# pranoyr/attention-models

Measured on AMD Instinct MI355X. Metric: ViTVQGAN 256px train-step images/sec, higher is better.
Workload: dtype f32; 1 GPU; BASELINE.json configs[2]: ViTVQGAN dim=256 patch=8 img=256 depth=6+6 h=8 d=64 mlp=2048 (SwiGLU), codebook 8192x32; GAN train step (D phase + G phase, gradient penalty, per_loss_weight=0), Adam, clip 1.0; global_batch=32, batch_per_gpu=32, parallelism=dp1

## Files before the change

### attention-models_amd/amk/lib.py

```python
import ctypes
import os
import re

_HERE = os.path.dirname(os.path.abspath(__file__))
LIB_PATH = os.environ.get("AMK_LIB") or os.path.join(_HERE, "libamk.so")
HEADER_PATH = os.path.normpath(os.path.join(_HERE, "..", "..", "include", "amk.h"))

AMK_OK = 0

_c = ctypes
_P = _c.c_void_p
_I = _c.c_int
_L = _c.c_int64
_F = _c.c_float



class GemmDesc(_c.Structure):
    _fields_ = [("op", _c.c_int32), ("epilogue", _c.c_int32), ("m", _L),
                ("n", _c.c_int32), ("k", _c.c_int32), ("split", _c.c_int32), ("reserved", _c.c_int32),
                ("a", _P), ("a2", _P), ("w", _P), ("w2", _P), ("c", _P), ("c2", _P),
                ("lda", _L), ("lda2", _L), ("ldw", _L), ("ldw2", _L), ("ldc", _L), ("ldc2", _L),
                ("bias", _P), ("bias2", _P), ("resid", _P), ("ldr", _L),
                ("ln_mean", _P), ("ln_rstd", _P), ("ln_gamma", _P), ("ln_beta", _P),
                ("ab", _P), ("ldab", _L), ("gate", _P), ("ldg", _L), ("dbias", _P)]


GEMM_NT, GEMM_NN, GEMM_TN = 0, 1, 2
EPI_BIAS, EPI_RESID, EPI_SWIGLU, EPI_SWIGLU_BWD = 0, 1, 2, 3

SIGNATURES = {
    "amk_version": (_I, []),
    "amk_arch": (_c.c_char_p, []),
    "amk_last_error": (_c.c_char_p, []),
    "amk_attn_fwd": (_I, [_P] * 7 + [_I] * 5 + [_L] * 12 + [_F, _P]),
    "amk_attn_scores_bytes": (_L, [_I, _I, _I, _I]),
    "amk_attn_fwd_keep": (_I, [_P] * 8 + [_I] * 5 + [_L] * 12 + [_F, _P]),
    "amk_attn_fwd_x6_ws_bytes": (_L, [_I, _I, _I]),
    "amk_attn_fwd_x6": (_I, [_P] * 8 + [_I] * 5 + [_L] * 12 + [_F, _P]),
    "amk_attn_bwd_ws_floats": (_L, [_I, _I, _I, _I, _I]),
    "amk_attn_bwd": (_I, [_P] * 12 + [_I] * 5 + [_L] * 24 + [_F, _I, _P]),
    "amk_attn_bwd_kept": (_I, [_P] * 13 + [_I] * 5 + [_L] * 24 + [_F, _I, _P]),
    "amk_vq_num_partials": (_L, [_L]),
    "amk_vq_lookup_fwd": (_I, [_P, _P, _L, _I, _I, _I] + [_P] * 9 + [_P]),
    "amk_vq_lookup_bwd": (_I, [_P] * 7 + [_F, _L, _I, _I, _P, _P, _P]),
    "amk_vq_lookup_bwd_rows": (_I, [_P] * 7 + [_F, _L, _I, _I, _P, _P, _P]),
    "amk_vq_padded_codes": (_I, [_I, _I]),
    "amk_vq_gather": (_I, [_P, _P, _L, _I, _I, _P, _P, _P]),
    "amk_agent_num_chunks": (_I, [_I]),
    "amk_agent_ws_floats": (_L, [_I, _I, _I, _I, _I]),
    "amk_agent_num_chunks_dh": (_I, [_I, _I]),
    "amk_agent_ws_floats_dh": (_L, [_I, _I, _I, _I, _I, _I]),
    "amk_agent_attn_fwd": (_I, [_P] * 10 + [_I] * 5 + [_L] * 12 + [_F, _P]),
    "amk_agent_attn_bwd": (_I, [_P] * 14 + [_I] * 5 + [_L] * 21 + [_F, _P]),
    "amk_agent_conv_grad_reduce": (_I, [_P, _P, _L, _I, _P, _P, _P]),
    "amk_rowsum_num_partials": (_I, [_L]),
    "amk_add_layernorm_fwd": (_I, [_P, _P, _P, _P, _L, _I, _F, _P, _P, _P, _P, _P]),
    "amk_add_layernorm_bwd": (_I, [_P, _P, _P, _P, _P, _P, _L, _I, _P, _P, _P]),
    "amk_colsum": (_I, [_P, _L, _I, _P, _P]),
    "amk_swiglu_fwd": (_I, [_P, _L, _I, _P, _P]),
    "amk_swiglu_bwd": (_I, [_P, _P, _L, _I, _P, _P]),
    "amk_geglu_fwd": (_I, [_P, _L, _I, _P, _P]),
    "amk_geglu_bwd": (_I, [_P, _P, _L, _I, _P, _P]),
    "amk_opt_num_partials": (_I, []),
    "amk_sumsq_partials": (_I, [_P, _L, _P, _P]),
    "amk_adam_flat_step": (_I, [_P] * 4 + [_L, _P, _P, _P, _I] + [_F] * 6 + [_I, _P, _P]),
    "amk_adam_flat_step_shadow": (_I, [_P] * 4 + [_L, _P, _P, _P, _I] + [_F] * 6 + [_I, _P, _P, _P]),
    "amk_gemm_x6_planes_bytes": (_L, [_I, _I]),
    "amk_gemm_x6_split": (_I, [_P, _L, _I, _I, _P, _P]),
    "amk_gemm_x6_nt": (_I, [_P, _L, _P, _P, _P, _L, _I, _I, _I, _P]),
    "amk_gemm_f32_ws_bytes": (_L, [_c.POINTER(GemmDesc)]),
    "amk_gemm_f32": (_I, [_c.POINTER(GemmDesc), _P, _L, _P]),
    "amk_row_stats": (_I, [_P, _L, _I, _F, _P, _P, _P]),
    "amk_attn_bf16_fwd": (_I, [_P] * 7 + [_I] * 5 + [_L] * 12 + [_F, _P]),
    "amk_attn_bf16_bwd_ws_floats": (_L, [_I, _I, _I, _I]),
    "amk_attn_bf16_bwd": (_I, [_P] * 12 + [_I] * 5 + [_L] * 24 + [_F, _P]),
    "amk_swiglu_bf16_fwd": (_I, [_P, _L, _I, _P, _P]),
    "amk_swiglu_bf16_bwd": (_I, [_P, _P, _L, _I, _P, _P]),
    "amk_add_layernorm_mixed_fwd": (_I, [_P, _I, _P, _P, _P, _L, _I, _F, _P, _P, _P, _P, _P]),
    "amk_add_layernorm_mixed_bwd": (_I, [_P, _I, _P, _P, _P, _P, _P, _L, _I, _P, _P, _P, _P]),
    "amk_gemm_bf16": (_I, [_I, _I, _P, _L, _P, _L, _P, _P, _L, _P, _L, _L, _I, _I, _P]),
    "amk_gemm_bf16_swiglu_bwd": (_I, [_P, _L, _P, _L, _P, _L, _P, _L, _L, _I, _I, _P]),
    "amk_gemm_tn_bf16_ws_bytes": (_L, [_L, _I, _I]),
    "amk_gemm_tn_bf16": (_I, [_P, _L, _P, _L, _P, _L, _P, _L, _I, _I, _P, _L, _P]),
    "amk_sample_step": (_I, [_P, _P, _F, _P, _c.c_uint64, _c.c_uint64, _F, _L, _I, _I, _P, _F, _P, _P, _P]),
    "amk_moe_route_ws_ints": (_L, [_L, _I, _I]),
    "amk_moe_route": (_I, [_P, _L, _I, _I] + [_P] * 8),
    "amk_grouped_gemm_nt": (_I, [_P, _L, _I, _P, _P, _P, _P, _L, _I, _I, _I, _P, _P]),
    "amk_grouped_gemm_nn": (_I, [_P, _L, _I, _P, _P, _P, _P, _L, _I, _I, _I, _P, _P]),
    "amk_grouped_gemm_nt_acc": (_I, [_P, _L, _I, _P, _P, _P, _P, _L, _I, _I, _I, _P, _I, _P]),
    "amk_grouped_gemm_nn_acc": (_I, [_P, _L, _I, _P, _P, _P, _P, _L, _I, _I, _I, _P, _I, _P]),
    "amk_grouped_gemm_wgrad": (_I, [_P, _L, _I, _P, _L, _I, _P, _P, _P, _L, _I, _I, _I, _P, _P, _P]),
    "amk_moe_combine": (_I, [_P, _P, _P, _L, _I, _I, _I, _P, _P]),
    "amk_moe_expert_sums": (_I, [_P, _L, _I, _P, _P, _L, _I, _I, _I, _P, _P]),
    "amk_moe_topk": (_I, [_P, _L, _I, _I, _P, _P, _P]),
    "amk_moe_route_distinct": (_I, [_P, _L, _I, _I, _P, _P, _P, _P]),
    "amk_moe_combine_rows": (_I, [_P, _P, _P, _L, _I, _I, _I, _I, _I, _P, _P]),
    "amk_moe_gate_grad_rows": (_I, [_P, _P, _P, _P, _L, _I, _I, _I, _I, _I, _P, _P]),
    "amk_moe_gate_grad": (_I, [_P, _P, _P, _P, _L, _I, _I, _I, _I, _P, _P]),
}

_lib = None


def declared_symbols(header_path=HEADER_PATH):
    text = open(header_path).read()
    text = re.sub(r"/\*.*?\*/", "", text, flags=re.S)
    return sorted(set(re.findall(r"\b(amk_[a-z0-9_]+)\s*\(", text)))


def load():
    global _lib
    if _lib is not None:
        return _lib
    if not os.path.exists(LIB_PATH):
        raise RuntimeError(
            f"{LIB_PATH} is missing: build it with `python -c 'import __graft_entry__ as g; g.build()'` "
            "(hipcc --offload-arch=gfx950). amk has no CPU or eager fallback."
        )
    lib = ctypes.CDLL(LIB_PATH)
    for name, (res, args) in SIGNATURES.items():
        fn = getattr(lib, name)
        fn.restype = res
        fn.argtypes = args
    arch = lib.amk_arch().decode()
    if arch != "gfx950":
        raise RuntimeError(f"libamk.so was built for {arch}, expected gfx950")
    _lib = lib
    return lib


def check(rc, what):
    if rc != AMK_OK:
        msg = load().amk_last_error().decode()
        raise RuntimeError(f"{what} failed with code {rc}: {msg}")
```

### attention-models_amd/amk/models/discriminator.py

```python
import contextlib

import torch
import torch.nn as nn
import torch.nn.functional as F
from torch.nn.grad import conv2d_input, conv2d_weight

_INPUT_GRAD_ONLY = False


@contextlib.contextmanager
def input_grad_only():
    global _INPUT_GRAD_ONLY
    old, _INPUT_GRAD_ONLY = _INPUT_GRAD_ONLY, True
    try:
        yield
    finally:
        _INPUT_GRAD_ONLY = old


class _ConvDataGrad(torch.autograd.Function):

    @staticmethod
    def forward(ctx, gy, weight, x_shape, stride, padding):
        ctx.save_for_backward(gy, weight)
        ctx.cfg = (stride, padding)
        return conv2d_input(x_shape, weight, gy, stride=stride, padding=padding)

    @staticmethod
    def backward(ctx, ggx):
        gy, weight = ctx.saved_tensors
        stride, padding = ctx.cfg
        ggx = ggx.contiguous()
        ggy = F.conv2d(ggx, weight, None, stride, padding) if ctx.needs_input_grad[0] else None
        gw = conv2d_weight(ggx, weight.shape, gy, stride=stride, padding=padding) if ctx.needs_input_grad[1] else None
        return ggy, gw, None, None, None


class _Conv(torch.autograd.Function):
    @staticmethod
    def forward(ctx, x, weight, bias, stride, padding):
        ctx.save_for_backward(x, weight)
        ctx.cfg = (stride, padding, bias is not None)
        return F.conv2d(x, weight, bias, stride, padding)

    @staticmethod
    def backward(ctx, gy):
        x, weight = ctx.saved_tensors
        stride, padding, has_bias = ctx.cfg
        gy = gy.contiguous()
        gx = _ConvDataGrad.apply(gy, weight, x.shape, stride, padding) if ctx.needs_input_grad[0] else None
        gw = gb = None
        if not _INPUT_GRAD_ONLY:
            if ctx.needs_input_grad[1]:
                gw = conv2d_weight(x, weight.shape, gy, stride=stride, padding=padding)
            if has_bias and ctx.needs_input_grad[2]:
                gb = gy.sum((0, 2, 3))
        return gx, gw, gb, None, None


class Conv2d(nn.Conv2d):

    def forward(self, x):
        if self.groups != 1 or self.dilation != (1, 1) or self.padding_mode != "zeros" or isinstance(self.padding, str):
            return super().forward(x)
        if torch.is_autocast_enabled():
            if self.in_channels < 8 and x.is_cuda:
                with torch.autocast("cuda", enabled=False):
                    return _Conv.apply(x.float(), self.weight, self.bias, self.stride, self.padding)
            return super().forward(x)
        return _Conv.apply(x, self.weight, self.bias, self.stride, self.padding)


class NLayerDiscriminator(nn.Module):
    def __init__(self, input_nc=3, ndf=64, n_layers=3):
        super().__init__()
        widths = [ndf * min(2 ** i, 8) for i in range(n_layers + 1)]
        layers = [Conv2d(input_nc, widths[0], 4, stride=2, padding=1), nn.LeakyReLU(0.2, True)]
        for i in range(1, n_layers + 1):
            stride = 2 if i < n_layers else 1
            layers += [
                Conv2d(widths[i - 1], widths[i], 4, stride=stride, padding=1, bias=False),
                nn.BatchNorm2d(widths[i]),
                nn.LeakyReLU(0.2, True),
            ]
        layers.append(Conv2d(widths[-1], 1, 4, stride=1, padding=1))
        self.model = nn.Sequential(*layers)

    def forward(self, x):
        return self.model(x)
```

### attention-models_amd/amk/ops.py

```python
import ctypes
import os
import weakref

import torch
from torch.autograd.function import once_differentiable

from . import lib as _lib

_NULL = ctypes.c_void_p(0)


def _ptr(t):
    return ctypes.c_void_p(t.data_ptr()) if t is not None else _NULL


def _stream():
    return ctypes.c_void_p(torch.cuda.current_stream().cuda_stream)


KERNEL_EVENTS = None


class _timed:

# ... 1106 lines not shown
        rc = L.amk_gemm_x6_nt(_ptr(a2), a2.stride(0), _ptr(planes), _ptr(bias), _ptr(c), N, M, N, K, _stream())
    _lib.check(rc, "amk_gemm_x6_nt")
    return c


def _x6_ok(x, weight):
    K = weight.shape[1]
    if K % 4 or x.numel() == 0 or x.data_ptr() % 16 or weight.data_ptr() % 16:
        return False
    if x.stride(-1) != 1 or (x.dim() >= 2 and x.stride(-2) % 4):
        return False
    return x.numel() * 4 < 0x7ffffff0 and weight.numel() * 8 < 0x7ffffff0


class _LinearX6(torch.autograd.Function):

    @staticmethod
    def forward(ctx, x, weight, bias):
        _require_device(x, weight, bias)
        x2 = x.reshape(-1, x.shape[-1])
        ctx.save_for_backward(x2, weight)
        ctx.x_shape = x.shape
        ctx.has_bias = bias is not None
        return gemm_x6_nt(x2, weight, bias).view(*x.shape[:-1], weight.shape[0])

    @staticmethod
    @once_differentiable
    def backward(ctx, dy):
        x2, weight = ctx.saved_tensors
        dy2 = dy.contiguous().view(-1, dy.shape[-1])
        dx = dw = db = None
        if ctx.needs_input_grad[0]:
            N = weight.shape[0]
            if N % 4 == 0:
                dx = gemm_x6_nt(dy2, weight.t().contiguous()).view(ctx.x_shape)
            else:
                dx = dy2.mm(weight).view(ctx.x_shape)
        if ctx.needs_input_grad[1]:
            dw = dy2.t().mm(x2)
        if ctx.has_bias and ctx.needs_input_grad[2]:
            db = colsum(dy2)
        return dx, dw, db


DENSE_MODE = os.environ.get("AMK_DENSE", "auto")


DENSE_AUTO_MAX_K = int(os.environ.get("AMK_DENSE_MAX_K", "512"))


def _dense_ok(x, *weights):
    if DENSE_MODE == "lib" or torch.is_autocast_enabled() or not x.is_cuda or x.dtype != torch.float32 or x.numel() == 0:
        return False
    if x.shape[-1] % 4 or x.shape[-1] < 128:
        return False
    if DENSE_MODE == "auto" and x.shape[-1] > DENSE_AUTO_MAX_K:
        return False
    return all(w.dtype == torch.float32 and w.shape[0] % 4 == 0 and w.shape[0] >= 128 and w.is_contiguous() for w in weights)


def _nn_plain(dy2, weight):
    from . import dense

    if DENSE_MODE == "amk":
        return dense.gemm_nn(dy2, weight)
    return dy2.mm(weight)


def _claim(p):
    ref = getattr(p, "_amk_reducer", None) if p is not None else None
    red = ref() if ref is not None else None
    if red is None:
        return None, None
    view = red.claim(p)
    return (red, view) if view is not None else (None, None)


class _DenseLinear(torch.autograd.Function):

    @staticmethod
    def forward(ctx, x, weight, bias):
        from . import dense

        x2 = x.reshape(-1, x.shape[-1])
        ctx.save_for_backward(x2, weight)
        ctx.x_shape = x.shape
        ctx.has_bias = bias is not None
        ctx.params = (weight, bias)
        if DENSE_MODE == "auto" and weight.shape[0] < 512:
            return torch.nn.functional.linear(x, weight, bias)
        return dense.gemm_nt(x2, weight, bias).view(*x.shape[:-1], weight.shape[0])

    @staticmethod
    @once_differentiable
    def backward(ctx, dy):
        from . import dense

        x2, weight = ctx.saved_tensors
        dy2 = dy.reshape(-1, dy.shape[-1])
        dx = dw = db = None
        if ctx.needs_input_grad[0]:
            dx = _nn_plain(dy2, weight).view(ctx.x_shape)
        if ctx.needs_input_grad[1] or (ctx.has_bias and ctx.needs_input_grad[2]):
            want_b = ctx.has_bias and ctx.needs_input_grad[2]
            (wr, wv), (br, bv) = _claim(ctx.params[0]), (_claim(ctx.params[1]) if want_b else (None, None))
            dw, _, db = dense.gemm_tn(dy2, x2, want_bias=want_b, out=wv, bias_out=bv)
            if wv is not None:
                wr.wrote(ctx.params[0])
                dw = None
            if bv is not None:
                br.wrote(ctx.params[1])
                db = None
        return dx, dw, db


def _tn_into(tn, y, x, weight, bias):
    (wr, wv), (br, bv) = _claim(weight), _claim(bias)
    res = tn(y, x, want_bias=bias is not None, out=wv, bias_out=bv)
    dw, db = res[0], res[-1]
    if wv is not None:
        wr.wrote(weight)
        dw = None
    if bv is not None:
        br.wrote(bias)
        db = None
    return dw, db


class _DenseLinear2(torch.autograd.Function):

    @staticmethod
    def forward(ctx, x, wa, wb):
        from . import dense

        x2 = x.reshape(-1, x.shape[-1])
        ctx.save_for_backward(x2, wa, wb)
        ctx.x_shape = x.shape
        ctx.params = (wa, wb)
        a, b = dense.gemm_nt(x2, wa, None, w2=wb)
        return a.view(*x.shape[:-1], wa.shape[0]), b.view(*x.shape[:-1], wb.shape[0])

    @staticmethod
    @once_differentiable
    def backward(ctx, da, db_):
        from . import dense

        x2, wa, wb = ctx.saved_tensors
        da2 = da.reshape(-1, da.shape[-1])
        db2 = db_.reshape(-1, db_.shape[-1])
        dx = dense.gemm_nn(da2, wa, a2=db2, w2=wb).view(ctx.x_shape) if ctx.needs_input_grad[0] else None
        dwa = dwb = None
        if ctx.needs_input_grad[1] or ctx.needs_input_grad[2]:
            (ar, av), (br, bv) = _claim(ctx.params[0]), _claim(ctx.params[1])
            dwa, dwb, _ = dense.gemm_tn(da2, x2, y2=db2, out=av, out2=bv)
            if av is not None:
                ar.wrote(ctx.params[0])
                dwa = None
            if bv is not None:
                br.wrote(ctx.params[1])
                dwb = None
        return dx, dwa, dwb


class _SwiGLUFFN(torch.autograd.Function):

    @staticmethod
    def forward(ctx, x, w12, b12, w3, b3):
        from . import dense

        x2 = x.reshape(-1, x.shape[-1])
        need = any(ctx.needs_input_grad)
        gate, ab = dense.gemm_nt_swiglu(x2, w12, b12, keep_ab=need)
        out = dense.gemm_nt(gate, w3, b3)
        if need:
            ctx.save_for_backward(x2, w12, w3, ab, gate)
        ctx.x_shape = x.shape
        ctx.has_bias = (b12 is not None, b3 is not None)
        ctx.params = (w12, b12, w3, b3)
        return out.view(*x.shape[:-1], w3.shape[0])

    @staticmethod
    @once_differentiable
    def backward(ctx, dout):
        from . import dense

        x2, w12, w3, ab, gate = ctx.saved_tensors
        d2 = dout.reshape(-1, dout.shape[-1])
        d_ab = dense.gemm_nn(d2, w3, swiglu_ab=ab)
        dw3, db3 = _tn_into(dense.gemm_tn, d2, gate, ctx.params[2], ctx.params[3] if ctx.has_bias[1] else None)
        dx = _nn_plain(d_ab, w12).view(ctx.x_shape) if ctx.needs_input_grad[0] else None
        dw12, db12 = _tn_into(dense.gemm_tn, d_ab, x2, ctx.params[0], ctx.params[1] if ctx.has_bias[0] else None)
        return dx, dw12, db12, dw3, db3


MIXED_WGRAD = os.environ.get("AMK_MIXED_WGRAD", "1") == "1"


def _w16(t):
    if t is None:
        return None
    shadow = getattr(t, "_amk_bf16", None)
    if shadow is not None and t._version == t._amk_bf16_version:
        return shadow
    return t.to(torch.bfloat16)


class _LinearMixed(torch.autograd.Function):

    @staticmethod
    def forward(ctx, x, weight, bias):
        x16, w16 = x.to(torch.bfloat16), _w16(weight)
        ctx.save_for_backward(x16, w16)
        ctx.has_bias, ctx.x_dtype = bias is not None, x.dtype
        ctx.params = (weight, bias)
        return torch.nn.functional.linear(x16, w16, _w16(bias))

    @staticmethod
    @once_differentiable
    def backward(ctx, dy):
        from . import dense

        x16, w16 = ctx.saved_tensors
        dy2 = dy.reshape(-1, dy.shape[-1])
        dx = dy2.mm(w16).view(x16.shape).to(ctx.x_dtype) if ctx.needs_input_grad[0] else None
        dw, db = _tn_into(dense.gemm_tn_bf16, dy2, x16.reshape(-1, x16.shape[-1]), ctx.params[0], ctx.params[1])
        return dx, dw, db


def _mixed_linear_ok(x, weight):
    return (MIXED_WGRAD and x.is_cuda and torch.get_autocast_dtype("cuda") == torch.bfloat16 and torch.is_grad_enabled()
            and weight.requires_grad and weight.dtype == torch.float32 and x.dtype in (torch.float32, torch.bfloat16)
            and weight.shape[0] % 8 == 0 and weight.shape[1] % 8 == 0 and x.numel() > 0)


def linear(x, weight, bias=None):
    if torch.is_autocast_enabled():
        if _mixed_linear_ok(x, weight):
            return _LinearMixed.apply(x, weight, bias)
        return torch.nn.functional.linear(x, weight, bias)
    if GEMM_MODE == "bf16x6" and _x6_ok(x, weight):
        return _LinearX6.apply(x, weight, bias)
    if _dense_ok(x, weight):
        return _DenseLinear.apply(x, weight, bias)
    if bias is None:
        return torch.nn.functional.linear(x, weight)
    return _BiasLinear.apply(x, weight, bias)


def linear2(x, wa, wb):
    if GEMM_MODE != "bf16x6" and _dense_ok(x, wa, wb) and wa.shape[0] % 128 == 0:
        return _DenseLinear2.apply(x, wa, wb)
    return linear(x, wa), linear(x, wb)


class _SwiGLUFFNMixed(torch.autograd.Function):

    @staticmethod
    def forward(ctx, x, w12, b12, w3, b3):
        from . import dense

        x16 = x.to(torch.bfloat16).reshape(-1, x.shape[-1])
        w12h, w3h = _w16(w12), _w16(w3)
        g, ab = dense.gemm_nt_swiglu_bf16(x16, w12h, b12)
        y = torch.nn.functional.linear(g, w3h, _w16(b3))
        ctx.save_for_backward(x16, ab, g, w12h, w3h)
        ctx.x_shape, ctx.x_dtype, ctx.bias = x.shape, x.dtype, (b12 is not None, b3 is not None)
        ctx.params = (w12, b12, w3, b3)
        return y.view(*x.shape[:-1], w3.shape[0])

    @staticmethod
    @once_differentiable
    def backward(ctx, dy):
        from . import dense

        x16, ab, g, w12h, w3h = ctx.saved_tensors
        dy2 = dy.reshape(-1, dy.shape[-1])
        dw3, db3 = _tn_into(dense.gemm_tn_bf16, dy2, g, ctx.params[2], ctx.params[3])
        dab = dense.gemm_nn_swiglu_bwd_bf16(dy2, w3h, ab)
        dw12, db12 = _tn_into(dense.gemm_tn_bf16, dab, x16, ctx.params[0], ctx.params[1])
        dx = dab.mm(w12h).view(ctx.x_shape).to(ctx.x_dtype) if ctx.needs_input_grad[0] else None
        return dx, dw12, db12, dw3, db3


def swiglu_ffn(x, w12, b12, w3, b3):
    if torch.is_autocast_enabled() and w12.shape[0] % 16 == 0 and w12.shape[0] >= 1024:
        if _mixed_linear_ok(x, w12) and _mixed_linear_ok(x, w3) and w3.requires_grad:
            with torch.autocast("cuda", enabled=False):
                return _SwiGLUFFNMixed.apply(x, w12, b12, w3, b3)
        no_grad = not torch.is_grad_enabled() or not any(
            t is not None and t.requires_grad for t in (x, w12, b12, w3, b3))
        if (MIXED_WGRAD and no_grad and x.is_cuda and torch.get_autocast_dtype("cuda") == torch.bfloat16
                and w12.dtype == torch.float32 and x.dtype in (torch.float32, torch.bfloat16) and w12.shape[1] % 8 == 0 and x.numel()):
            from . import dense

            g, _ = dense.gemm_nt_swiglu_bf16(x.to(torch.bfloat16).reshape(-1, x.shape[-1]), _w16(w12), b12, keep_ab=False)
            return torch.nn.functional.linear(g, _w16(w3), _w16(b3)).view(*x.shape[:-1], w3.shape[0])
    if GEMM_MODE != "bf16x6" and _dense_ok(x, w12) and w3.shape[1] % 4 == 0 and w3.shape[0] % 4 == 0 and w3.is_contiguous():
        return _SwiGLUFFN.apply(x, w12, b12, w3, b3)
    ab = linear(x, w12, b12)
    if ab.shape[-1] % 8 == 0:
        return linear(swiglu(ab), w3, b3)
    a, b = ab.chunk(2, dim=-1)
    return linear(torch.nn.functional.silu(a) * b, w3, b3)
```

### include/amk.h

```cpp
#ifndef AMK_H_
#define AMK_H_

#include <stdint.h>

#ifdef __cplusplus
extern "C" {
#endif

#define AMK_VERSION 140

enum {
  AMK_OK = 0,
  AMK_EINVAL = -1,
  AMK_EUNSUPPORTED = -2,
  AMK_ELAUNCH = -3
};

int amk_version(void);
const char* amk_arch(void);
const char* amk_last_error(void);

int amk_attn_fwd(const float* q, const float* k, const float* v, float* o, float* stats,
                 const uint8_t* key_mask, const uint8_t* causal_mask,
                 int B, int H, int I, int J, int D,
                 int64_t q_sb, int64_t q_st, int64_t q_sh,
                 int64_t k_sb, int64_t k_st, int64_t k_sh,
                 int64_t v_sb, int64_t v_st, int64_t v_sh,
                 int64_t o_sb, int64_t o_st, int64_t o_sh,
                 float scale, void* stream);

int64_t amk_attn_scores_bytes(int B, int H, int I, int J);
int amk_attn_fwd_keep(const float* q, const float* k, const float* v, float* o, float* stats, float* scores,
                      const uint8_t* key_mask, const uint8_t* causal_mask,
                      int B, int H, int I, int J, int D,
                      int64_t q_sb, int64_t q_st, int64_t q_sh,
                      int64_t k_sb, int64_t k_st, int64_t k_sh,
                      int64_t v_sb, int64_t v_st, int64_t v_sh,
                      int64_t o_sb, int64_t o_st, int64_t o_sh,
                      float scale, void* stream);

int64_t amk_attn_fwd_x6_ws_bytes(int B, int H, int J);
int amk_attn_fwd_x6(const float* q, const float* k, const float* v, float* o, float* stats, void* ws,
                    const uint8_t* key_mask, const uint8_t* causal_mask,
                    int B, int H, int I, int J, int D,
                    int64_t q_sb, int64_t q_st, int64_t q_sh,
                    int64_t k_sb, int64_t k_st, int64_t k_sh,
                    int64_t v_sb, int64_t v_st, int64_t v_sh,
                    int64_t o_sb, int64_t o_st, int64_t o_sh,
                    float scale, void* stream);

#define AMK_ATTN_BWD_DELTA 1
#define AMK_ATTN_BWD_DKDV 2
#define AMK_ATTN_BWD_DQ 4
#define AMK_ATTN_BWD_FUSED 8
#define AMK_ATTN_BWD_ALL 7
#define AMK_ATTN_BWD_FAST 9
#define AMK_ATTN_BWD_KEYS128 16
#define AMK_ATTN_BWD_KEYS256 32
#define AMK_ATTN_BWD_DQ_REPRO 64
#define AMK_ATTN_BWD_FAST_REPRO 73
int64_t amk_attn_bwd_ws_floats(int B, int H, int I, int J, int stages);
int amk_attn_bwd(const float* q, const float* k, const float* v, const float* o,
                 const float* stats, const float* d_o,
                 float* dq, float* dk, float* dv, float* delta_ws,
                 const uint8_t* key_mask, const uint8_t* causal_mask,
                 int B, int H, int I, int J, int D,
                 int64_t q_sb, int64_t q_st, int64_t q_sh,
                 int64_t k_sb, int64_t k_st, int64_t k_sh,
                 int64_t v_sb, int64_t v_st, int64_t v_sh,
                 int64_t o_sb, int64_t o_st, int64_t o_sh,
                 int64_t do_sb, int64_t do_st, int64_t do_sh,
                 int64_t dq_sb, int64_t dq_st, int64_t dq_sh,
                 int64_t dk_sb, int64_t dk_st, int64_t dk_sh,
                 int64_t dv_sb, int64_t dv_st, int64_t dv_sh,
                 float scale, int stages, void* stream);
int amk_attn_bwd_kept(const float* scores, const float* q, const float* k, const float* v, const float* o,
                      const float* stats, const float* d_o,
                      float* dq, float* dk, float* dv, float* delta_ws,
                      const uint8_t* key_mask, const uint8_t* causal_mask,
                      int B, int H, int I, int J, int D,
                      int64_t q_sb, int64_t q_st, int64_t q_sh,
                      int64_t k_sb, int64_t k_st, int64_t k_sh,
                      int64_t v_sb, int64_t v_st, int64_t v_sh,
                      int64_t o_sb, int64_t o_st, int64_t o_sh,
                      int64_t do_sb, int64_t do_st, int64_t do_sh,
                      int64_t dq_sb, int64_t dq_st, int64_t dq_sh,
                      int64_t dk_sb, int64_t dk_st, int64_t dk_sh,
                      int64_t dv_sb, int64_t dv_st, int64_t dv_sh,
                      float scale, int stages, void* stream);

int64_t amk_vq_num_partials(int64_t N);
int amk_vq_padded_codes(int K, int nsplit);
int amk_vq_lookup_fwd(const float* z, const float* codebook, int64_t N, int K, int C, int nsplit,
                      float* en_ws, float* ee_ws, float* pmin_ws, int32_t* pidx_ws,
                      int64_t* idx, float* out, float* zq, float* zn, float* sqerr_partial,
                      void* stream);

int amk_vq_lookup_bwd(const float* z, const float* codebook, const float* zn, const float* zq,
                      const int64_t* idx, const float* g_out, const float* g_loss, float beta,
                      int64_t N, int K, int C, float* dz, float* dcodebook, void* stream);

int amk_vq_lookup_bwd_rows(const float* z, const float* codebook, const float* zn, const float* zq,
                           const int64_t* idx, const float* g_out, const float* g_loss, float beta,
                           int64_t N, int K, int C, float* dz, float* ge_rows, void* stream);

int amk_vq_gather(const int64_t* idx, const float* codebook, int64_t N, int K, int C,
                  float* out, int32_t* bad_count, void* stream);


int64_t amk_moe_route_ws_ints(int64_t U, int E, int k);
int amk_moe_route(const float* logits, int64_t U, int E, int k,
                  int64_t* ids, float* gate, int32_t* counts, int32_t* rank, int32_t* blockhist,
                  int32_t* offsets, int32_t* perm, void* stream);

int amk_grouped_gemm_nt(const float* A, int64_t lda, int a_div, const float* W, const float* bias,
                        const int32_t* offsets, const int32_t* perm, int64_t P, int E, int N, int Kd,
                        float* Y, void* stream);

int amk_grouped_gemm_nn(const float* A, int64_t lda, int a_div, const float* W, const float* scale,
                        const int32_t* offsets, const int32_t* perm, int64_t P, int E, int N, int Kd,
                        float* Y, void* stream);

int amk_grouped_gemm_nt_acc(const float* A, int64_t lda, int a_div, const float* W, const float* bias,
                            const int32_t* offsets, const int32_t* perm, int64_t P, int E, int N, int Kd,
                            float* Y, int y_div, void* stream);
int amk_grouped_gemm_nn_acc(const float* A, int64_t lda, int a_div, const float* W, const float* scale,
                            const int32_t* offsets, const int32_t* perm, int64_t P, int E, int N, int Kd,
                            float* Y, int y_div, void* stream);

int amk_grouped_gemm_wgrad(const float* G, int64_t ldg, int g_div, const float* X, int64_t ldx, int x_div,
                           const float* scale, const int32_t* offsets, const int32_t* perm,
                           int64_t P, int E, int N, int Kd, float* dW, float* dbias, void* stream);

int amk_moe_combine(const float* Y, const int64_t* ids, const float* scale, int64_t G, int outer, int k,
                    int N, float* out, void* stream);

int amk_moe_topk(const float* logits, int64_t U, int E, int k, int64_t* ids, float* gate, void* stream);

int amk_moe_route_distinct(const int64_t* ids, int64_t G, int fan, int E, uint64_t* mask,
                           int32_t* offsets, int32_t* perm, void* stream);

int amk_moe_combine_rows(const float* Y, const int64_t* ids, const float* scale, int64_t G, int outer, int k,
                         int N, int v_div, int E, float* out, void* stream);
int amk_moe_gate_grad_rows(const float* d_out, const float* Y, const int64_t* ids, const float* gate,
                           int64_t P, int k, int E, int N, int g_div, int v_div, float* dlogits, void* stream);

int amk_moe_expert_sums(const float* A, int64_t lda, int a_div, const int64_t* ids, const float* scale,
                        int64_t G, int fan, int E, int d, float* Z, void* stream);

int amk_moe_gate_grad(const float* d_out, const float* Y, const int64_t* ids, const float* gate,
                      int64_t P, int k, int E, int N, int g_div, float* dlogits, void* stream);

int amk_agent_num_chunks(int T);
int64_t amk_agent_ws_floats(int B, int H, int T, int P, int backward);
int amk_agent_num_chunks_dh(int T, int D);
int64_t amk_agent_ws_floats_dh(int B, int H, int T, int P, int D, int backward);

int amk_agent_attn_fwd(const float* q, const float* k, const float* v, const float* conv_w, const float* conv_b,
                       float* o, float* agents, float* vagent, float* stats1, float* ws,
                       int B, int H, int T, int D, int P,
                       int64_t q_sb, int64_t q_st, int64_t q_sh, int64_t k_sb, int64_t k_st, int64_t k_sh,
                       int64_t v_sb, int64_t v_st, int64_t v_sh, int64_t o_sb, int64_t o_st, int64_t o_sh,
                       float scale, void* stream);

int amk_agent_attn_bwd(const float* q, const float* k, const float* v, const float* conv_w, const float* d_o,
                       const float* agents, const float* vagent, const float* stats1,
                       float* dq, float* dk, float* dv, float* ws, float* dconvw_part, float* dconvb_part,
                       int B, int H, int T, int D, int P,
                       int64_t q_sb, int64_t q_st, int64_t q_sh, int64_t k_sb, int64_t k_st, int64_t k_sh,
                       int64_t v_sb, int64_t v_st, int64_t v_sh, int64_t do_sb, int64_t do_st, int64_t do_sh,
                       int64_t dq_sb, int64_t dq_st, int64_t dq_sh, int64_t dk_sb, int64_t dk_st, int64_t dk_sh,
                       int64_t dv_sb, int64_t dv_st, int64_t dv_sh, float scale, void* stream);

int amk_agent_conv_grad_reduce(const float* dconvw_part, const float* dconvb_part, int64_t rows, int D,
                               float* dconvw, float* dconvb, void* stream);

int amk_rowsum_num_partials(int64_t M);
int amk_add_layernorm_fwd(const float* x, const float* res, const float* gamma, const float* beta,
                          int64_t M, int D, float eps, float* h, float* y, float* mean, float* rstd, void* stream);
int amk_add_layernorm_bwd(const float* dy, const float* h, const float* dh_in, const float* gamma,
                          const float* mean, const float* rstd, int64_t M, int D, float* dh, float* dgb_part,
                          void* stream);
int amk_colsum(const float* x, int64_t M, int N, float* part, void* stream);

int amk_swiglu_fwd(const float* ab, int64_t M, int H, float* out, void* stream);
int amk_swiglu_bwd(const float* ab, const float* d_out, int64_t M, int H, float* d_ab, void* stream);

int amk_geglu_fwd(const float* ab, int64_t M, int H, float* out, void* stream);
int amk_geglu_bwd(const float* ab, const float* d_out, int64_t M, int H, float* d_ab, void* stream);

int amk_opt_num_partials(void);
int amk_sumsq_partials(const float* x, int64_t n, float* partials, void* stream);
int amk_adam_flat_step(float* param, float* grad, float* exp_avg, float* exp_avg_sq, int64_t n,
                       const int32_t* seg_param, const float* param_tab,
                       const float* partials, int n_partials,
                       float max_norm, float lr, float beta1, float beta2, float eps, float weight_decay,
                       int decoupled, float* norm_out, void* stream);
int amk_adam_flat_step_shadow(float* param, float* grad, float* exp_avg, float* exp_avg_sq, int64_t n,
                              const int32_t* seg_param, const float* param_tab,
                              const float* partials, int n_partials,
                              float max_norm, float lr, float beta1, float beta2, float eps, float weight_decay,
                              int decoupled, float* norm_out, void* param_bf16, void* stream);

int amk_sample_step(const float* logits, const float* null_logits, float cfg_scale,
                    const float* gumbel, uint64_t seed, uint64_t offset, float tau,
                    int64_t R, int V, int keep, const uint8_t* mask, float unmasked_score,
                    int64_t* ids, float* scores, void* stream);

int64_t amk_gemm_x6_planes_bytes(int N, int K);
int amk_gemm_x6_split(const float* W, int64_t ldw, int N, int K, void* planes, void* stream);
int amk_gemm_x6_nt(const float* A, int64_t lda, const void* w_planes, const float* bias,
                   float* C, int64_t ldc, int M, int N, int K, void* stream);

enum { AMK_GEMM_NT = 0, AMK_GEMM_NN = 1, AMK_GEMM_TN = 2 };
enum { AMK_EPI_BIAS = 0, AMK_EPI_RESID = 1, AMK_EPI_SWIGLU = 2, AMK_EPI_SWIGLU_BWD = 3 };
typedef struct amk_gemm_desc {
  int32_t op, epilogue;
  int64_t m;
  int32_t n, k, split, reserved;
  const float *a, *a2, *w, *w2;
  float *c, *c2;
  int64_t lda, lda2, ldw, ldw2, ldc, ldc2;
  const float *bias, *bias2, *resid;
  int64_t ldr;
  const float *ln_mean, *ln_rstd, *ln_gamma, *ln_beta;
  const float* ab;
  int64_t ldab;
  float* gate;
  int64_t ldg;
  float* dbias;
} amk_gemm_desc;
int64_t amk_gemm_f32_ws_bytes(const amk_gemm_desc* d);
int amk_gemm_f32(const amk_gemm_desc* d, void* workspace, int64_t ws_bytes, void* stream);
int amk_row_stats(const float* x, int64_t M, int D, float eps, float* mean, float* rstd, void* stream);

int amk_attn_bf16_fwd(const void* q, const void* k, const void* v, void* o, float* stats,
                      const uint8_t* key_mask, const uint8_t* causal_mask,
                      int B, int H, int I, int J, int D,
                      int64_t q_sb, int64_t q_st, int64_t q_sh, int64_t k_sb, int64_t k_st, int64_t k_sh,
                      int64_t v_sb, int64_t v_st, int64_t v_sh, int64_t o_sb, int64_t o_st, int64_t o_sh,
                      float scale, void* stream);
int64_t amk_attn_bf16_bwd_ws_floats(int B, int H, int I, int J);
int amk_attn_bf16_bwd(const void* q, const void* k, const void* v, const void* o, const float* stats, const void* d_o,
                      void* dq, void* dk, void* dv, float* ws,
                      const uint8_t* key_mask, const uint8_t* causal_mask,
                      int B, int H, int I, int J, int D,
                      int64_t q_sb, int64_t q_st, int64_t q_sh, int64_t k_sb, int64_t k_st, int64_t k_sh,
                      int64_t v_sb, int64_t v_st, int64_t v_sh, int64_t o_sb, int64_t o_st, int64_t o_sh,
                      int64_t do_sb, int64_t do_st, int64_t do_sh, int64_t dq_sb, int64_t dq_st, int64_t dq_sh,
                      int64_t dk_sb, int64_t dk_st, int64_t dk_sh, int64_t dv_sb, int64_t dv_st, int64_t dv_sh,
                      float scale, void* stream);

int amk_swiglu_bf16_fwd(const void* ab, int64_t M, int H, void* out, void* stream);
int amk_swiglu_bf16_bwd(const void* ab, const void* d_out, int64_t M, int H, void* d_ab, void* stream);
int amk_add_layernorm_mixed_fwd(const void* x, int x_is_bf16, const float* res, const float* gamma, const float* beta,
                                int64_t M, int D, float eps, float* h, void* y_bf16, float* mean, float* rstd, void* stream);
int amk_add_layernorm_mixed_bwd(const void* dy, int dy_is_bf16, const float* h, const float* dh_in, const float* gamma,
                                const float* mean, const float* rstd, int64_t M, int D, float* dh, void* dh_bf16,
                                float* dgb_part, void* stream);

int64_t amk_gemm_tn_bf16_ws_bytes(int64_t M, int N, int K);
int amk_gemm_tn_bf16(const void* y, int64_t ldy, const void* x, int64_t ldx, float* c, int64_t ldc, float* dbias,
                     int64_t M, int N, int K, void* workspace, int64_t ws_bytes, void* stream);

int amk_gemm_bf16(int op, int epi, const void* a, int64_t lda, const void* w, int64_t ldw, const float* bias,
                  void* c, int64_t ldc, void* g, int64_t ldg, int64_t M, int N, int K, void* stream);

int amk_gemm_bf16_swiglu_bwd(const void* dy, int64_t lddy, const void* w3, int64_t ldw, const void* ab, int64_t ldab,
                             void* dab, int64_t lddab, int64_t M, int H, int K, void* stream);

#ifdef __cplusplus
}
#endif
#endif
```

Measured before the change: 297.0 images/s.

## Fuse discriminator BatchNorm and LeakyReLU into custom HIP kernels with double-backward

Adds fused BatchNorm2d+LeakyReLU forward, backward and double-backward HIP kernels (two-pass segmented per-channel reductions) and routes discriminator BN→LeakyReLU pairs through them by default. It targets the separate PyTorch/MIOpen BN and activation kernels and their autograd double-backward graph used by the gradient penalty. In exchange it adds custom reduction code, extra workspace allocations per call, and numerical-parity risk in the second-order gradients.

```diff
diff --git a/attention-models_amd/amk/lib.py b/attention-models_amd/amk/lib.py
--- a/attention-models_amd/amk/lib.py
+++ b/attention-models_amd/amk/lib.py
@@ -98,6 +98,10 @@
     "amk_moe_combine_rows": (_I, [_P, _P, _P, _L, _I, _I, _I, _I, _I, _P, _P]),
     "amk_moe_gate_grad_rows": (_I, [_P, _P, _P, _P, _L, _I, _I, _I, _I, _I, _P, _P]),
     "amk_moe_gate_grad": (_I, [_P, _P, _P, _P, _L, _I, _I, _I, _I, _P, _P]),
+    "amk_bnact_ws_floats": (_L, [_I, _I, _L]),
+    "amk_bnact_fwd": (_I, [_P, _P, _P, _I, _I, _L, _F, _F, _F] + [_P] * 7),
+    "amk_bnact_bwd": (_I, [_P] * 6 + [_I, _I, _L, _F] + [_P] * 6),
+    "amk_bnact_bwd_bwd": (_I, [_P] * 10 + [_I, _I, _L, _F] + [_P] * 5),
 }
 
 _lib = None
diff --git a/attention-models_amd/amk/models/discriminator.py b/attention-models_amd/amk/models/discriminator.py
--- a/attention-models_amd/amk/models/discriminator.py
+++ b/attention-models_amd/amk/models/discriminator.py
@@ -4,6 +4,8 @@
 import torch.nn as nn
 import torch.nn.functional as F
 from torch.nn.grad import conv2d_input, conv2d_weight
+
+from .. import ops
 
 _INPUT_GRAD_ONLY = False
 
@@ -16,6 +18,10 @@
         yield
     finally:
         _INPUT_GRAD_ONLY = old
+
+
+def input_grad_only_active():
+    return _INPUT_GRAD_ONLY
 
 
 class _ConvDataGrad(torch.autograd.Function):
@@ -87,4 +93,17 @@
         self.model = nn.Sequential(*layers)
 
     def forward(self, x):
-        return self.model(x)
+        if ops.discr_norm_mode() != "amk":
+            return self.model(x)
+        layers = list(self.model)
+        i = 0
+        while i < len(layers):
+            m = layers[i]
+            nxt = layers[i + 1] if i + 1 < len(layers) else None
+            if isinstance(m, nn.BatchNorm2d) and isinstance(nxt, nn.LeakyReLU) and ops.bn_leaky_relu_ok(m, x):
+                x = ops.bn_leaky_relu(x, m, nxt.negative_slope)
+                i += 2
+            else:
+                x = m(x)
+                i += 1
+        return x
diff --git a/attention-models_amd/amk/ops.py b/attention-models_amd/amk/ops.py
--- a/attention-models_amd/amk/ops.py
+++ b/attention-models_amd/amk/ops.py
@@ -1432,3 +1432,106 @@
         return linear(swiglu(ab), w3, b3)
     a, b = ab.chunk(2, dim=-1)
     return linear(torch.nn.functional.silu(a) * b, w3, b3)
+
+
+def discr_norm_mode():
+    return os.environ.get("AMK_DISCR_NORM", "amk")
+
+
+def _bn_aligned(t):
+    t = t.contiguous()
+    return t if t.data_ptr() % 16 == 0 else t.clone()
+
+
+def _bn_dims(x):
+    N, C, H, W = x.shape
+    return N, C, H * W
+
+
+def _bn_ws(x):
+    N, C, HW = _bn_dims(x)
+    return torch.empty(int(_lib.load().amk_bnact_ws_floats(N, C, HW)), device=x.device, dtype=torch.float32)
+
+
+class _BNActGrad(torch.autograd.Function):
+
+    @staticmethod
+    def forward(ctx, gz, x, weight, bias, mean, rstd, slope):
+        gz = _bn_aligned(gz)
+        N, C, HW = _bn_dims(x)
+        L = _lib.load()
+        gx = torch.empty_like(x)
+        sums = torch.empty((2, C), device=x.device, dtype=torch.float32)
+        dw = torch.empty_like(weight)
+        db = torch.empty_like(bias)
+        _lib.check(L.amk_bnact_bwd(_ptr(gz), _ptr(x), _ptr(weight), _ptr(bias), _ptr(mean), _ptr(rstd), N, C, HW,
+                                   float(slope), _ptr(gx), _ptr(sums), _ptr(dw), _ptr(db), _ptr(_bn_ws(x)), _stream()),
+                   "amk_bnact_bwd")
+        ctx.save_for_backward(gz, x, weight, bias, mean, rstd, sums)
+        ctx.slope = slope
+        ctx.set_materialize_grads(False)
+        return gx, dw, db
+
+    @staticmethod
+    @once_differentiable
+    def backward(ctx, ggx, ggw, ggb):
+        gz, x, weight, bias, mean, rstd, sums = ctx.saved_tensors
+        if ggx is None and ggw is None and ggb is None:
+            return None, None, None, None, None, None, None
+        ggx = torch.zeros_like(x) if ggx is None else _bn_aligned(ggx)
+        N, C, HW = _bn_dims(x)
+        g_gz = torch.empty_like(x)
+        g_x = torch.empty_like(x)
+        g_w = torch.empty_like(weight) if ctx.needs_input_grad[2] else None
+        _lib.check(_lib.load().amk_bnact_bwd_bwd(
+            _ptr(ggx), _ptr(ggw.contiguous() if ggw is not None else None), _ptr(ggb.contiguous() if ggb is not None else None),
+            _ptr(gz), _ptr(x), _ptr(weight), _ptr(bias), _ptr(mean), _ptr(rstd), _ptr(sums), N, C, HW, float(ctx.slope),
+            _ptr(g_gz), _ptr(g_x), _ptr(g_w), _ptr(_bn_ws(x)), _stream()), "amk_bnact_bwd_bwd")
+        return (g_gz if ctx.needs_input_grad[0] else None, g_x if ctx.needs_input_grad[1] else None, g_w,
+                None, None, None, None)
+
+
+class _BNAct(torch.autograd.Function):
+
+    @staticmethod
+    def forward(ctx, x, weight, bias, running_mean, running_var, eps, momentum, slope):
+        N, C, HW = _bn_dims(x)
+        L = _lib.load()
+        z = torch.empty_like(x)
+        mean = torch.empty(C, device=x.device, dtype=torch.float32)
+        rstd = torch.empty(C, device=x.device, dtype=torch.float32)
+        _lib.check(L.amk_bnact_fwd(_ptr(x), _ptr(weight), _ptr(bias), N, C, HW, float(eps), float(momentum), float(slope),
+                                   _ptr(z), _ptr(mean), _ptr(rstd), _ptr(running_mean), _ptr(running_var),
+                                   _ptr(_bn_ws(x)), _stream()), "amk_bnact_fwd")
+        ctx.save_for_backward(x, weight, bias, mean, rstd)
+        ctx.slope = slope
+        ctx.set_materialize_grads(False)
+        return z
+
+    @staticmethod
+    def backward(ctx, gz):
+        if gz is None:
+            return (None,) * 8
+        x, weight, bias, mean, rstd = ctx.saved_tensors
+        from .models.discriminator import input_grad_only_active
+
+        gx, dw, db = _BNActGrad.apply(gz, x, weight, bias, mean, rstd, ctx.slope)
+        if input_grad_only_active():
+            dw = db = None
+        return (gx if ctx.needs_input_grad[0] else None, dw if ctx.needs_input_grad[1] else None,
+                db if ctx.needs_input_grad[2] else None, None, None, None, None, None)
+
+
+def bn_leaky_relu_ok(bn, x):
+    return (bn.training and bn.track_running_stats and bn.affine and bn.momentum is not None
+            and bn.running_mean is not None and x.is_cuda and x.dtype == torch.float32 and x.dim() == 4
+            and x.is_contiguous() and x.numel() > 0 and x.shape[0] * x.shape[2] * x.shape[3] > 1
+            and not torch.is_autocast_enabled() and bn.weight.dtype == torch.float32)
+
+
+def bn_leaky_relu(x, bn, slope):
+    _require_device(x, bn.weight, bn.bias)
+    if bn.num_batches_tracked is not None:
+        bn.num_batches_tracked.add_(1)
+    return _BNAct.apply(_bn_aligned(x), bn.weight, bn.bias, bn.running_mean, bn.running_var, bn.eps, bn.momentum,
+                        float(slope))
diff --git a/attention-models_amd/csrc/discr_norm.hip b/attention-models_amd/csrc/discr_norm.hip
--- /dev/null
+++ b/attention-models_amd/csrc/discr_norm.hip
@@ -0,0 +1,422 @@
+#include "amk_common.h"
+
+namespace amk_bn {
+
+constexpr int BLOCK = 256;
+constexpr int WAVES = BLOCK / 64;
+constexpr int64_t SEG = 4096;
+
+struct Geo {
+  int N, C;
+  int64_t HW;
+  int PP;
+  int Q;
+  int64_t L;
+  int S;
+};
+
+static Geo make_geo(int N, int C, int64_t HW) {
+  Geo g;
+  g.N = N; g.C = C; g.HW = HW;
+  if (HW <= SEG) {
+    g.PP = (int)(SEG / HW);
+    if (g.PP > N) g.PP = N;
+    g.Q = 1; g.L = HW;
+    g.S = (N + g.PP - 1) / g.PP;
+  } else {
+    g.PP = 1;
+    g.Q = (int)((HW + SEG - 1) / SEG);
+    g.L = (((HW + g.Q - 1) / g.Q) + 3) & ~(int64_t)3;
+    g.S = N * g.Q;
+  }
+  return g;
+}
+
+struct Seg {
+  int p0, p1;
+  int64_t e0, e1;
+};
+
+__device__ __forceinline__ Seg seg_of(const Geo& g, int s) {
+  Seg r;
+  if (g.Q == 1) {
+    r.p0 = s * g.PP; r.p1 = min(g.N, r.p0 + g.PP);
+    r.e0 = 0; r.e1 = g.HW;
+  } else {
+    r.p0 = s / g.Q; r.p1 = r.p0 + 1;
+    r.e0 = min(g.HW, (int64_t)(s % g.Q) * g.L);
+    r.e1 = min(g.HW, r.e0 + g.L);
+  }
+  return r;
+}
+
+__device__ __forceinline__ float seg_count(const Geo& g, int s) {
+  const Seg r = seg_of(g, s);
+  return (float)((int64_t)(r.p1 - r.p0) * (r.e1 - r.e0));
+}
+
+template <int W> struct Width { static constexpr int value = W; };
+
+template <int W>
+__device__ __forceinline__ void ld(const float* p, float (&v)[W]) {
+  if constexpr (W == 4) {
+    const float4 t = *reinterpret_cast<const float4*>(p);
+    v[0] = t.x; v[1] = t.y; v[2] = t.z; v[3] = t.w;
+  } else {
+    v[0] = *p;
+  }
+}
+
+template <int W>
+__device__ __forceinline__ void st(float* p, const float (&v)[W]) {
+  if constexpr (W == 4) *reinterpret_cast<float4*>(p) = make_float4(v[0], v[1], v[2], v[3]);
+  else *p = v[0];
+}
+
+template <class F>
+__device__ __forceinline__ void seg_walk(const Geo& g, int c, int s, F&& f) {
+  const Seg r = seg_of(g, s);
+  const int64_t len = r.e1 - r.e0;
+  const int t = threadIdx.x;
+  for (int p = r.p0; p < r.p1; ++p) {
+    const int64_t base = ((int64_t)p * g.C + c) * g.HW + r.e0;
+    const int head = (int)min((int64_t)((4 - (base & 3)) & 3), len);
+    const int64_t nv = (len - head) >> 2;
+    const int tail = (int)(len - head - 4 * nv);
+    for (int64_t i = t; i < nv; i += BLOCK) f(Width<4>{}, base + head + 4 * i);
+    if (t < head) f(Width<1>{}, base + t);
+    else if (t < head + tail) f(Width<1>{}, base + 4 * nv + t);
+  }
+}
+
+struct Sum {
+  template <int K>
+  __device__ __forceinline__ void operator()(float (&a)[K], const float (&b)[K]) const {
+#pragma unroll
+    for (int k = 0; k < K; ++k) a[k] += b[k];
+  }
+};
+
+struct Chan {
+  __device__ __forceinline__ void operator()(float (&a)[3], const float (&b)[3]) const {
+    const float n = a[0] + b[0];
+    if (b[0] == 0.f) return;
+    if (a[0] == 0.f) { a[0] = b[0]; a[1] = b[1]; a[2] = b[2]; return; }
+    const float d = b[1] - a[1], f = b[0] / n;
+    a[1] += d * f;
+    a[2] += b[2] + d * d * a[0] * f;
+    a[0] = n;
+  }
+};
+
+template <int K, class Op>
+__device__ __forceinline__ void block_reduce(float (&v)[K], Op op, float* lds) {
+  const int lane = threadIdx.x & 63, wave = threadIdx.x >> 6;
+#pragma unroll
+  for (int o = 32; o >= 1; o >>= 1) {
+    float w[K];
+#pragma unroll
+    for (int k = 0; k < K; ++k) w[k] = __shfl_xor(v[k], o, 64);
+    op(v, w);
+  }
+  if (lane == 0) {
+#pragma unroll
+    for (int k = 0; k < K; ++k) lds[wave * K + k] = v[k];
+  }
+  __syncthreads();
+#pragma unroll
+  for (int k = 0; k < K; ++k) v[k] = lds[k];
+#pragma unroll
+  for (int w = 1; w < WAVES; ++w) {
+    float u[K];
+#pragma unroll
+    for (int k = 0; k < K; ++k) u[k] = lds[w * K + k];
+    op(v, u);
+  }
+  __syncthreads();
+}
+
+template <int K>
+__device__ __forceinline__ void fold_sums(const float* __restrict__ part, const Geo& g, int c, float (&v)[K],
+                                          float* lds) {
+#pragma unroll
+  for (int k = 0; k < K; ++k) v[k] = 0.f;
+  for (int j = threadIdx.x; j < g.S; j += BLOCK) {
+#pragma unroll
+    for (int k = 0; k < K; ++k) v[k] += part[((int64_t)c * g.S + j) * K + k];
+  }
+  block_reduce<K>(v, Sum{}, lds);
+}
+
+__global__ __launch_bounds__(BLOCK) void stats_kernel(const float* __restrict__ x, Geo g, float* __restrict__ part) {
+  __shared__ float lds[WAVES * 3];
+  const int s = blockIdx.x, c = blockIdx.y;
+  float v[1] = {0.f};
+  seg_walk(g, c, s, [&](auto w, int64_t off) {
+    constexpr int W = decltype(w)::value;
+    float xv[W];
+    ld<W>(x + off, xv);
+#pragma unroll
+    for (int k = 0; k < W; ++k) v[0] += xv[k];
+  });
+  block_reduce<1>(v, Sum{}, lds);
+  const float cnt = seg_count(g, s);
+  const float mean = cnt > 0.f ? v[0] / cnt : 0.f;
+  float q[1] = {0.f};
+  seg_walk(g, c, s, [&](auto w, int64_t off) {
+    constexpr int W = decltype(w)::value;
+    float xv[W];
+    ld<W>(x + off, xv);
+#pragma unroll
+    for (int k = 0; k < W; ++k) { const float d = xv[k] - mean; q[0] += d * d; }
+  });
+  block_reduce<1>(q, Sum{}, lds);
+  if (threadIdx.x == 0) {
+    part[((int64_t)c * g.S + s) * 2] = mean;
+    part[((int64_t)c * g.S + s) * 2 + 1] = q[0];
+  }
+}
+
+__global__ __launch_bounds__(BLOCK) void fwd_apply_kernel(
+    const float* __restrict__ x, const float* __restrict__ gamma, const float* __restrict__ beta, Geo g,
+    const float* __restrict__ part, float eps, float momentum, float slope, float* __restrict__ z,
+    float* __restrict__ mean_out, float* __restrict__ rstd_out, float* __restrict__ run_mean,
+    float* __restrict__ run_var) {
+  __shared__ float lds[WAVES * 3];
+  const int s = blockIdx.x, c = blockIdx.y;
+  float a[3] = {0.f, 0.f, 0.f};
+  for (int j = threadIdx.x; j < g.S; j += BLOCK) {
+    const float b[3] = {seg_count(g, j), part[((int64_t)c * g.S + j) * 2], part[((int64_t)c * g.S + j) * 2 + 1]};
+    Chan{}(a, b);
+  }
+  block_reduce<3>(a, Chan{}, lds);
+  const float n = a[0], mu = a[1], var = a[2] / n;
+  const float r = rsqrtf(var + eps);
+  const float scale = gamma[c] * r, shift = beta[c] - mu * scale;
+  if (s == 0 && threadIdx.x == 0) {
+    mean_out[c] = mu;
+    rstd_out[c] = r;
+    if (run_mean) run_mean[c] = (1.f - momentum) * run_mean[c] + momentum * mu;
+    if (run_var) run_var[c] = (1.f - momentum) * run_var[c] + momentum * (a[2] / (n - 1.f));
+  }
+  seg_walk(g, c, s, [&](auto w, int64_t off) {
+    constexpr int W = decltype(w)::value;
+    float xv[W];
+    ld<W>(x + off, xv);
+#pragma unroll
+    for (int k = 0; k < W; ++k) {
+      const float y = fmaf(xv[k], scale, shift);
+      xv[k] = y > 0.f ? y : slope * y;
+    }
+    st<W>(z + off, xv);
+  });
+}
+
+struct Chn {
+  float mu, r, scale, shift;
+};
+
+__device__ __forceinline__ Chn chn(const float* gamma, const float* beta, const float* mean, const float* rstd, int c) {
+  Chn h;
+  h.mu = mean[c]; h.r = rstd[c];
+  h.scale = gamma[c] * h.r;
+  h.shift = beta[c] - h.mu * h.scale;
+  return h;
+}
+
+__global__ __launch_bounds__(BLOCK) void bwd_reduce_kernel(
+    const float* __restrict__ gz, const float* __restrict__ x, const float* __restrict__ gamma,
+    const float* __restrict__ beta, const float* __restrict__ mean, const float* __restrict__ rstd, Geo g, float slope,
+    float* __restrict__ part) {
+  __shared__ float lds[WAVES * 3];
+  const int s = blockIdx.x, c = blockIdx.y;
+  const Chn h = chn(gamma, beta, mean, rstd, c);
+  float v[2] = {0.f, 0.f};
+  seg_walk(g, c, s, [&](auto w, int64_t off) {
+    constexpr int W = decltype(w)::value;
+    float xv[W], gv[W];
+    ld<W>(x + off, xv);
+    ld<W>(gz + off, gv);
+#pragma unroll
+    for (int k = 0; k < W; ++k) {
+      const float gy = fmaf(xv[k], h.scale, h.shift) > 0.f ? gv[k] : slope * gv[k];
+      v[0] += gy;
+      v[1] += gy * ((xv[k] - h.mu) * h.r);
+    }
+  });
+  block_reduce<2>(v, Sum{}, lds);
+  if (threadIdx.x == 0) {
+    part[((int64_t)c * g.S + s) * 2] = v[0];
+    part[((int64_t)c * g.S + s) * 2 + 1] = v[1];
+  }
+}
+
+__global__ __launch_bounds__(BLOCK) void bwd_apply_kernel(
+    const float* __restrict__ gz, const float* __restrict__ x, const float* __restrict__ gamma,
+    const float* __restrict__ beta, const float* __restrict__ mean, const float* __restrict__ rstd, Geo g, float slope,
+    const float* __restrict__ part, float* __restrict__ gx, float* __restrict__ sums, float* __restrict__ dgamma,
+    float* __restrict__ dbeta) {
+  __shared__ float lds[WAVES * 3];
+  const int s = blockIdx.x, c = blockIdx.y;
+  const Chn h = chn(gamma, beta, mean, rstd, c);
+  float v[2];
+  fold_sums<2>(part, g, c, v, lds);
+  if (s == 0 && threadIdx.x == 0) {
+    sums[c] = v[0];
+    sums[g.C + c] = v[1];
+    if (dbeta) dbeta[c] = v[0];
+    if (dgamma) dgamma[c] = v[1];
+  }
+  const float inv_n = 1.f / (float)((double)g.N * (double)g.HW);
+  const float A = v[0] * inv_n, B = v[1] * inv_n;
+  seg_walk(g, c, s, [&](auto w, int64_t off) {
+    constexpr int W = decltype(w)::value;
+    float xv[W], gv[W];
+    ld<W>(x + off, xv);
+    ld<W>(gz + off, gv);
+#pragma unroll
+    for (int k = 0; k < W; ++k) {
+      const float gy = fmaf(xv[k], h.scale, h.shift) > 0.f ? gv[k] : slope * gv[k];
+      const float xh = (xv[k] - h.mu) * h.r;
+      xv[k] = h.scale * (gy - A - xh * B);
+    }
+    st<W>(gx + off, xv);
+  });
+}
+
+__global__ __launch_bounds__(BLOCK) void bwd_bwd_reduce_kernel(
+    const float* __restrict__ ggx, const float* __restrict__ gz, const float* __restrict__ x,
+    const float* __restrict__ gamma, const float* __restrict__ beta, const float* __restrict__ mean,
+    const float* __restrict__ rstd, Geo g, float slope, float* __restrict__ part) {
+  __shared__ float lds[WAVES * 3];
+  const int s = blockIdx.x, c = blockIdx.y;
+  const Chn h = chn(gamma, beta, mean, rstd, c);
+  float v[3] = {0.f, 0.f, 0.f};
+  seg_walk(g, c, s, [&](auto w, int64_t off) {
+    constexpr int W = decltype(w)::value;
+    float xv[W], gv[W], qv[W];
+    ld<W>(x + off, xv);
+    ld<W>(gz + off, gv);
+    ld<W>(ggx + off, qv);
+#pragma unroll
+    for (int k = 0; k < W; ++k) {
+      const float gy = fmaf(xv[k], h.scale, h.shift) > 0.f ? gv[k] : slope * gv[k];
+      v[0] += qv[k];
+      v[1] += qv[k] * ((xv[k] - h.mu) * h.r);
+      v[2] += qv[k] * gy;
+    }
+  });
+  block_reduce<3>(v, Sum{}, lds);
+  if (threadIdx.x == 0) {
+#pragma unroll
+    for (int k = 0; k < 3; ++k) part[((int64_t)c * g.S + s) * 3 + k] = v[k];
+  }
+}
+
+__global__ __launch_bounds__(BLOCK) void bwd_bwd_apply_kernel(
+    const float* __restrict__ ggx, const float* __restrict__ gg_gamma, const float* __restrict__ gg_beta,
+    const float* __restrict__ gz, const float* __restrict__ x, const float* __restrict__ gamma,
+    const float* __restrict__ beta, const float* __restrict__ mean, const float* __restrict__ rstd,
+    const float* __restrict__ sums, Geo g, float slope, const float* __restrict__ part, float* __restrict__ g_gz,
+    float* __restrict__ g_x, float* __restrict__ g_gamma) {
+  __shared__ float lds[WAVES * 3];
+  const int s = blockIdx.x, c = blockIdx.y;
+  const Chn h = chn(gamma, beta, mean, rstd, c);
+  float v[3];
+  fold_sums<3>(part, g, c, v, lds);
+  const float n = (float)((double)g.N * (double)g.HW), inv_n = 1.f / n;
+  const float A = sums[c] * inv_n, B = sums[g.C + c] * inv_n;
+  const float Cc = v[0] * inv_n, D = v[1] * inv_n, E = v[2] * inv_n;
+  const float ggg = gg_gamma ? gg_gamma[c] : 0.f, ggb = gg_beta ? gg_beta[c] : 0.f;
+  if (s == 0 && threadIdx.x == 0 && g_gamma) g_gamma[c] = n * h.r * (E - A * Cc - B * D);
+  const float k1 = E - A * Cc - 3.f * B * D;
+  const float gr2 = h.scale * h.r;
+  const float gr = ggg * h.r;
+  seg_walk(g, c, s, [&](auto w, int64_t off) {
+    constexpr int W = decltype(w)::value;
+    float xv[W], gv[W], qv[W];
+    ld<W>(x + off, xv);
+    ld<W>(gz + off, gv);
+    ld<W>(ggx + off, qv);
+#pragma unroll
+    for (int k = 0; k < W; ++k) {
+      const bool pos = fmaf(xv[k], h.scale, h.shift) > 0.f;
+      const float gy = pos ? gv[k] : slope * gv[k];
+      const float xh = (xv[k] - h.mu) * h.r;
+      const float q = qv[k] - Cc;
+      const float t = h.scale * (q - xh * D) + ggg * xh + ggb;
+      gv[k] = pos ? t : slope * t;
+      xv[k] = gr * (gy - A - xh * B) - gr2 * (xh * k1 + B * q + D * (gy - A));
+    }
+    st<W>(g_gz + off, gv);
+    st<W>(g_x + off, xv);
+  });
+}
+
+}
+
+using namespace amk_bn;
+
+static bool a16(const void* p) { return (reinterpret_cast<uintptr_t>(p) & 15) == 0; }
+
+#define AMK_BN_SHAPE(what)                                                                       \
+  AMK_CHECK_ARG(N > 0 && C > 0 && HW > 0, what ": non-positive size");                           \
+  AMK_CHECK_SUPPORTED(C <= 65535 && (int64_t)N * HW <= ((int64_t)1 << 31),                       \
+                      what ": shape N %d C %d HW %lld not supported", N, C, (long long)HW)
+
+extern "C" int64_t amk_bnact_ws_floats(int N, int C, int64_t HW) {
+  if (N <= 0 || C <= 0 || HW <= 0) return 0;
+  return (int64_t)C * make_geo(N, C, HW).S * 3;
+}
+
+extern "C" int amk_bnact_fwd(const float* x, const float* gamma, const float* beta, int N, int C, int64_t HW,
+                             float eps, float momentum, float slope, float* z, float* mean, float* rstd,
+                             float* running_mean, float* running_var, float* ws, void* stream) {
+  AMK_CHECK_ARG(x && gamma && beta && z && mean && rstd && ws, "amk_bnact_fwd: null pointer");
+  AMK_BN_SHAPE("amk_bnact_fwd");
+  AMK_CHECK_ARG(N * HW > 1, "amk_bnact_fwd: a channel needs more than one value");
+  AMK_CHECK_ARG(a16(x) && a16(z), "amk_bnact_fwd: x and z must be 16-byte aligned");
+  hipStream_t st = static_cast<hipStream_t>(stream);
+  const Geo g = make_geo(N, C, HW);
+  const dim3 grid(g.S, C), block(BLOCK);
+  hipLaunchKernelGGL(stats_kernel, grid, block, 0, st, x, g, ws);
+  hipLaunchKernelGGL(fwd_apply_kernel, grid, block, 0, st, x, gamma, beta, g, ws, eps, momentum, slope, z, mean, rstd,
+                     running_mean, running_var);
+  AMK_CHECK_LAUNCH("amk_bnact_fwd");
+  return AMK_OK;
+}
+
+extern "C" int amk_bnact_bwd(const float* gz, const float* x, const float* gamma, const float* beta,
+                             const float* mean, const float* rstd, int N, int C, int64_t HW, float slope, float* gx,
+                             float* sums, float* dgamma, float* dbeta, float* ws, void* stream) {
+  AMK_CHECK_ARG(gz && x && gamma && beta && mean && rstd && gx && sums && ws, "amk_bnact_bwd: null pointer");
+  AMK_BN_SHAPE("amk_bnact_bwd");
+  AMK_CHECK_ARG(a16(gz) && a16(x) && a16(gx), "amk_bnact_bwd: gz, x and gx must be 16-byte aligned");
+  hipStream_t st = static_cast<hipStream_t>(stream);
+  const Geo g = make_geo(N, C, HW);
+  const dim3 grid(g.S, C), block(BLOCK);
+  hipLaunchKernelGGL(bwd_reduce_kernel, grid, block, 0, st, gz, x, gamma, beta, mean, rstd, g, slope, ws);
+  hipLaunchKernelGGL(bwd_apply_kernel, grid, block, 0, st, gz, x, gamma, beta, mean, rstd, g, slope, ws, gx, sums,
+                     dgamma, dbeta);
+  AMK_CHECK_LAUNCH("amk_bnact_bwd");
+  return AMK_OK;
+}
+
+extern "C" int amk_bnact_bwd_bwd(const float* ggx, const float* gg_gamma, const float* gg_beta, const float* gz,
+                                 const float* x, const float* gamma, const float* beta, const float* mean,
+                                 const float* rstd, const float* sums, int N, int C, int64_t HW, float slope,
+                                 float* g_gz, float* g_x, float* g_gamma, float* ws, void* stream) {
+  AMK_CHECK_ARG(ggx && gz && x && gamma && beta && mean && rstd && sums && g_gz && g_x && ws,
+                "amk_bnact_bwd_bwd: null pointer");
+  AMK_BN_SHAPE("amk_bnact_bwd_bwd");
+  AMK_CHECK_ARG(a16(ggx) && a16(gz) && a16(x) && a16(g_gz) && a16(g_x),
+                "amk_bnact_bwd_bwd: ggx, gz, x, g_gz and g_x must be 16-byte aligned");
+  hipStream_t st = static_cast<hipStream_t>(stream);
+  const Geo g = make_geo(N, C, HW);
+  const dim3 grid(g.S, C), block(BLOCK);
+  hipLaunchKernelGGL(bwd_bwd_reduce_kernel, grid, block, 0, st, ggx, gz, x, gamma, beta, mean, rstd, g, slope, ws);
+  hipLaunchKernelGGL(bwd_bwd_apply_kernel, grid, block, 0, st, ggx, gg_gamma, gg_beta, gz, x, gamma, beta, mean, rstd,
+                     sums, g, slope, ws, g_gz, g_x, g_gamma);
+  AMK_CHECK_LAUNCH("amk_bnact_bwd_bwd");
+  return AMK_OK;
+}
diff --git a/include/amk.h b/include/amk.h
--- a/include/amk.h
+++ b/include/amk.h
@@ -269,6 +269,18 @@
 int amk_gemm_bf16_swiglu_bwd(const void* dy, int64_t lddy, const void* w3, int64_t ldw, const void* ab, int64_t ldab,
                              void* dab, int64_t lddab, int64_t M, int H, int K, void* stream);
 
+int64_t amk_bnact_ws_floats(int N, int C, int64_t HW);
+int amk_bnact_fwd(const float* x, const float* gamma, const float* beta, int N, int C, int64_t HW, float eps,
+                  float momentum, float slope, float* z, float* mean, float* rstd, float* running_mean,
+                  float* running_var, float* ws, void* stream);
+int amk_bnact_bwd(const float* gz, const float* x, const float* gamma, const float* beta, const float* mean,
+                  const float* rstd, int N, int C, int64_t HW, float slope, float* gx, float* sums, float* dgamma,
+                  float* dbeta, float* ws, void* stream);
+int amk_bnact_bwd_bwd(const float* ggx, const float* gg_gamma, const float* gg_beta, const float* gz, const float* x,
+                      const float* gamma, const float* beta, const float* mean, const float* rstd, const float* sums,
+                      int N, int C, int64_t HW, float slope, float* g_gz, float* g_x, float* g_gamma, float* ws,
+                      void* stream);
+
 #ifdef __cplusplus
 }
 #endif
```

Result: faster. 306.2 images/s, median of 6 (+3.1%).
